# zefanyang/pacingpseudo

Hardware: AMD Instinct MI355X
Metric: training images/sec (256x256, 5-class) (higher is better)
Workload: dtype f32 (matrix products as 3 fp16 MFMA products of split operands with fp32 accumulation, or fp32 MFMA)

## Files before the change

### pacingpseudo_amd/csrc/pp_wino.hip

```cpp
#include "pp_common.h"
#include <stdlib.h>

PP_NS_BEGIN

typedef float f32x16 __attribute__((ext_vector_type(16)));
typedef float f32x4 __attribute__((ext_vector_type(4)));
#define WLD 36
#define WBK 32

struct WinoGeom {
  int N, H, W, dil;
  int Hs, Ws;
  int m;
  int th, tw;
  int T;
  int nb;
};
static inline int wino_tile(int H, int W, int dil) {
  return (H % (4 * dil) == 0 && W % (4 * dil) == 0) ? 4 : 2;
}
static inline WinoGeom wino_geom(int N, int H, int W, int dil) {
  const int m = wino_tile(H, W, dil);
  WinoGeom g{N, H, W, dil, H / dil, W / dil, m, H / dil / m, W / dil / m, 0, (m + 2) * (m + 2)};
  g.T = N * dil * dil * g.th * g.tw;
// ... 707 lines not shown
      U[(r * 4 + 3) * plane + at] = t[r][2];
    }
  }
}

struct GemmArgs {
  const float* A; const float* B; float* C;
  int M, N, K;
  int m_tiles, n_tiles;
  unsigned a_bytes, b_bytes;
  int nb;
};

template <int TM, int TN, int WAVES_M, int WAVES_N>
__global__ __launch_bounds__(WAVES_M* WAVES_N * 64) void wino_gemm_kernel(GemmArgs a) {
  constexpr int NT = WAVES_M * WAVES_N * 64;
  constexpr int BM = 32 * TM * WAVES_M, BN = 32 * TN * WAVES_N;
  constexpr int RPP = NT / 8;
  constexpr int A_PASSES = BM / RPP, B_PASSES = BN / RPP;
  extern __shared__ __attribute__((aligned(16))) float smem[];
  float* As = smem;
  float* Bs = smem + 2 * BM * WLD;
  const int tid = threadIdx.x, lane = tid & 63, wv = tid >> 6;
  const int wm = wv / WAVES_N, wn = wv % WAVES_N;
  const int lr = lane & 31, lh = lane >> 5;
  const int q = tid & 7, r0 = tid >> 3;
  const int per_batch = a.m_tiles * a.n_tiles;
  int b = blockIdx.x;
  const int total = per_batch * a.nb;
  if ((total & 7) == 0) b = (b & 7) * (total >> 3) + (b >> 3);
  const int batch = b / per_batch;
  const int rem = b - batch * per_batch;
  const int mt = rem / a.n_tiles, nt = rem % a.n_tiles;
  const int m0 = mt * BM, n0 = nt * BN;
  const float* Ab = a.A + (size_t)batch * a.M * a.K;
  const float* Bb = a.B + (size_t)batch * a.N * a.K;
  const __amdgpu_buffer_rsrc_t rs_a = __builtin_amdgcn_make_buffer_rsrc((void*)Ab, 0, a.a_bytes, 0x00020000);
  const __amdgpu_buffer_rsrc_t rs_b = __builtin_amdgcn_make_buffer_rsrc((void*)Bb, 0, a.b_bytes, 0x00020000);
  f32x4 ra[A_PASSES], rb[B_PASSES];
  const int n_it = (a.K + WBK - 1) / WBK;
  auto load_tile = [&](int it) {
    const int c = it * WBK + q * 4;
    const int cok = (int)(c < a.K);
#pragma unroll
    for (int i = 0; i < A_PASSES; ++i) {
      const int m = m0 + r0 + i * RPP;
      const unsigned off = (cok & (int)(m < a.M)) ? (unsigned)(m * a.K + c) * 4u : 0xffffffffu;
      ra[i] = __builtin_bit_cast(f32x4, __builtin_amdgcn_raw_buffer_load_b128(rs_a, off, 0, 0));
    }
#pragma unroll
    for (int i = 0; i < B_PASSES; ++i) {
      const int n = n0 + r0 + i * RPP;
      const unsigned off = (cok & (int)(n < a.N)) ? (unsigned)(n * a.K + c) * 4u : 0xffffffffu;
      rb[i] = __builtin_bit_cast(f32x4, __builtin_amdgcn_raw_buffer_load_b128(rs_b, off, 0, 0));
    }
  };
  auto store_tile = [&](int buf) {
#pragma unroll
    for (int i = 0; i < A_PASSES; ++i)
      *reinterpret_cast<f32x4*>(As + buf * BM * WLD + (r0 + i * RPP) * WLD + q * 4) = ra[i];
#pragma unroll
    for (int i = 0; i < B_PASSES; ++i)
      *reinterpret_cast<f32x4*>(Bs + buf * BN * WLD + (r0 + i * RPP) * WLD + q * 4) = rb[i];
  };
  f32x16 acc[TM][TN];
#pragma unroll
  for (int i = 0; i < TM; ++i)
#pragma unroll
    for (int j = 0; j < TN; ++j)
#pragma unroll
      for (int r = 0; r < 16; ++r) acc[i][j][r] = 0.f;
  load_tile(0);
  store_tile(0);
  __syncthreads();
  for (int it = 0; it < n_it; ++it) {
    const int buf = it & 1;
    const bool more = it + 1 < n_it;
    const float* Ap = As + buf * BM * WLD + (wm * TM * 32 + lr) * WLD + lh * 4;
    const float* Bp = Bs + buf * BN * WLD + (wn * TN * 32 + lr) * WLD + lh * 4;
    float4 af[2][TM], bf[2][TN];
    auto read_frags = [&](int kk, int slot) {
#pragma unroll
      for (int i = 0; i < TM; ++i) af[slot][i] = *reinterpret_cast<const float4*>(Ap + i * 32 * WLD + kk * 8);
#pragma unroll
      for (int j = 0; j < TN; ++j) bf[slot][j] = *reinterpret_cast<const float4*>(Bp + j * 32 * WLD + kk * 8);
    };
    auto mfma_block = [&](int slot) {
#pragma unroll
      for (int i = 0; i < TM; ++i)
#pragma unroll
        for (int j = 0; j < TN; ++j) {
          acc[i][j] = __builtin_amdgcn_mfma_f32_32x32x2f32(af[slot][i].x, bf[slot][j].x, acc[i][j], 0, 0, 0);
          acc[i][j] = __builtin_amdgcn_mfma_f32_32x32x2f32(af[slot][i].y, bf[slot][j].y, acc[i][j], 0, 0, 0);
          acc[i][j] = __builtin_amdgcn_mfma_f32_32x32x2f32(af[slot][i].z, bf[slot][j].z, acc[i][j], 0, 0, 0);
          acc[i][j] = __builtin_amdgcn_mfma_f32_32x32x2f32(af[slot][i].w, bf[slot][j].w, acc[i][j], 0, 0, 0);
        }
    };
    read_frags(0, 0);
    read_frags(1, 1);
    __builtin_amdgcn_sched_barrier(0);
    mfma_block(0);
    __builtin_amdgcn_sched_barrier(0);
    if (more) load_tile(it + 1);
    read_frags(2, 0);
    __builtin_amdgcn_sched_barrier(0);
    mfma_block(1);
    __builtin_amdgcn_sched_barrier(0);
    read_frags(3, 1);
    __builtin_amdgcn_sched_barrier(0);
    mfma_block(0);
    __builtin_amdgcn_sched_barrier(0);
    if (more) store_tile(buf ^ 1);
    __builtin_amdgcn_sched_barrier(0);
    mfma_block(1);
    __syncthreads();
  }
  float* Cb = a.C + (size_t)batch * a.M * a.N;
#pragma unroll
  for (int j = 0; j < TN; ++j) {
    const int n = n0 + (wn * TN + j) * 32 + lr;
    if (n >= a.N) continue;
#pragma unroll
    for (int i = 0; i < TM; ++i)
#pragma unroll
      for (int r = 0; r < 16; ++r) {
        const int m = m0 + (wm * TM + i) * 32 + (r & 3) + 8 * (r >> 2) + 4 * lh;
        if (m < a.M) Cb[(size_t)m * a.N + n] = acc[i][j][r];
      }
  }
}

template <int TM, int TN, int WAVES_M, int WAVES_N>
static int launch_gemm(GemmArgs a, hipStream_t s) {
  constexpr int BM = 32 * TM * WAVES_M, BN = 32 * TN * WAVES_N;
  a.m_tiles = pp_cdiv(a.M, BM);
  a.n_tiles = pp_cdiv(a.N, BN);
  const size_t lds = (size_t)2 * (BM + BN) * WLD * sizeof(float);
  auto kern = wino_gemm_kernel<TM, TN, WAVES_M, WAVES_N>;
  {
    pp_max_lds(reinterpret_cast<const void*>(kern), (int)lds);
  }
  hipLaunchKernelGGL(kern, dim3(a.nb * a.m_tiles * a.n_tiles), dim3(WAVES_M * WAVES_N * 64), lds, s, a);
  return pp_launch_status("wino_gemm");
}

struct GemmPsArgs {
  const char* A; const char* B; float* C;
  int M, N, K;
  int m_tiles, n_tiles, nb;
  unsigned a_bytes, b_bytes;
  const float* a_amax; float a_bound;
};

__device__ __forceinline__ f32x16 ps_mfma(f16x8 a, f16x8 b, f32x16 c, int) { return __builtin_amdgcn_mfma_f32_32x32x16_f16(a, b, c, 0, 0, 0); }

template <int TM, int TN, int WAVES_M, int WAVES_N, bool X1>
__global__ __launch_bounds__(WAVES_M* WAVES_N * 64) __attribute__((amdgpu_waves_per_eu(WAVES_M* WAVES_N / 4)))
void wino_gemm_ps_kernel(GemmPsArgs a) {
  constexpr int NW = WAVES_M * WAVES_N;
  constexpr int BM = 32 * TM * WAVES_M, BN = 32 * TN * WAVES_N;
  constexpr int STAGE = (BM + BN) * 128;
  constexpr int FA = BM / 8 / NW, FB = BN / 8 / NW;
  static_assert((BM / 8) % NW == 0 && (BN / 8) % NW == 0, "tile rows must split evenly over the waves");
  extern __shared__ __attribute__((aligned(1024))) char smem_ps[];
  typedef __attribute__((address_space(3))) void* lds_ptr;
  const int tid = threadIdx.x, lane = tid & 63;
  const int wv = __builtin_amdgcn_readfirstlane(tid >> 6);
  const int wm = wv / WAVES_N, wn = wv % WAVES_N;
  const int lr = lane & 31, lh = lane >> 5;
  const int per_batch = a.m_tiles * a.n_tiles;
  int b = blockIdx.x;
  const int total = per_batch * a.nb;
  if ((total & 7) == 0) b = (b & 7) * (total >> 3) + (b >> 3);
  const int batch = b / per_batch;
  const int rem = b - batch * per_batch;
  const int mt = rem / a.n_tiles, nt = rem % a.n_tiles;
  const int m0 = mt * BM, n0 = nt * BN;
  float s_in, s_out;
  ps_scales(a.a_amax, a.a_bound, s_in, s_out);
  const __amdgpu_buffer_rsrc_t rs_a = __builtin_amdgcn_make_buffer_rsrc((void*)(a.A + (size_t)batch * a.a_bytes), 0, a.a_bytes, 0x00020000);
  const __amdgpu_buffer_rsrc_t rs_b = __builtin_amdgcn_make_buffer_rsrc((void*)(a.B + (size_t)batch * a.b_bytes), 0, a.b_bytes, 0x00020000);
  const int fr = lane >> 3, fq = lane & 7;
  const unsigned kbytes = (unsigned)a.K * 4u;
  unsigned offA[FA], offB[FB], pcA[FA], pcB[FB];
#pragma unroll
  for (int f = 0; f < FA; ++f) {
    const int row = (f * NW + wv) * 8 + fr;
    pcA[f] = (unsigned)((fq ^ ((row >> 1) & 7)) * 16);
    offA[f] = (m0 + row < a.M) ? (unsigned)(m0 + row) * kbytes + pcA[f] : 0xffffffffu;
  }
#pragma unroll
  for (int f = 0; f < FB; ++f) {
    const int row = (f * NW + wv) * 8 + fr;
    pcB[f] = (unsigned)((fq ^ ((row >> 1) & 7)) * 16);
    offB[f] = (n0 + row < a.N) ? (unsigned)(n0 + row) * kbytes + pcB[f] : 0xffffffffu;
  }
  auto fill_one = [&](int f, int it, int stage) {
    char* base = smem_ps + stage * STAGE + wv * 1024;
    const unsigned koff = (unsigned)it * 128u;
    if (f < FA) {
      const unsigned o = (offA[f < FA ? f : 0] != 0xffffffffu && koff + pcA[f < FA ? f : 0] < kbytes) ? offA[f < FA ? f : 0] + koff : 0xffffffffu;
      __builtin_amdgcn_raw_ptr_buffer_load_lds(rs_a, (lds_ptr)(base + f * NW * 1024), 16, o, 0, 0, 0);
    } else {
      const int g = f - FA < FB ? f - FA : 0;
      const unsigned o = (offB[g] != 0xffffffffu && koff + pcB[g] < kbytes) ? offB[g] + koff : 0xffffffffu;
      __builtin_amdgcn_raw_ptr_buffer_load_lds(rs_b, (lds_ptr)(base + BM * 128 + g * NW * 1024), 16, o, 0, 0, 0);
    }
  };
  auto fill = [&](int it, int stage) {
#pragma unroll
    for (int f = 0; f < FA + FB; ++f) fill_one(f, it, stage);
  };
  f32x16 accm[TM][TN], accc[TM][TN];
#pragma unroll
  for (int i = 0; i < TM; ++i)
#pragma unroll
    for (int j = 0; j < TN; ++j)
#pragma unroll
      for (int r = 0; r < 16; ++r) { accm[i][j][r] = 0.f; accc[i][j][r] = 0.f; }
  const int sw = (lr >> 1) & 7;
  int qo[2][2];
#pragma unroll
  for (int kb = 0; kb < 2; ++kb)
#pragma unroll
    for (int part = 0; part < 2; ++part) qo[kb][part] = ((4 * kb + 2 * lh + part) ^ sw) * 16;
  const int a_row = (wm * TM * 32 + lr) * 128, b_row = BM * 128 + (wn * TN * 32 + lr) * 128;
  const int n_it = (a.K + 31) / 32;
  f16x8 ah[2][TM], al[2][TM], bh[2][TN], bl[2][TN];
  auto read_half = [&](int kb, int stage) {
    const char* Ap = smem_ps + stage * STAGE + a_row;
    const char* Bp = smem_ps + stage * STAGE + b_row;
#pragma unroll
    for (int i = 0; i < TM; ++i) {
      ah[kb][i] = *reinterpret_cast<const f16x8*>(Ap + i * 32 * 128 + qo[kb][0]);
      if (!X1) al[kb][i] = *reinterpret_cast<const f16x8*>(Ap + i * 32 * 128 + qo[kb][1]);
    }
#pragma unroll
    for (int j = 0; j < TN; ++j) {
      bh[kb][j] = *reinterpret_cast<const f16x8*>(Bp + j * 32 * 128 + qo[kb][0]);
      if (!X1) bl[kb][j] = *reinterpret_cast<const f16x8*>(Bp + j * 32 * 128 + qo[kb][1]);
    }
  };
  auto wait_landed = [&]() {
    asm volatile("s_waitcnt vmcnt(%0) lgkmcnt(0)" ::"n"(FA + FB) : "memory");
    __builtin_amdgcn_s_barrier();
    asm volatile("" ::: "memory");
  };
  static_assert(FA + FB <= 16, "the counted wait assumes a handful of DMAs per wave and stage");
  fill(0, 0);
  fill(1, 1);
  asm volatile("s_waitcnt vmcnt(%0)" ::"n"(FA + FB) : "memory");
  __builtin_amdgcn_s_barrier();
  asm volatile("" ::: "memory");
  fill(2, 2);
  read_half(0, 0);
  read_half(1, 0);
  int st_next = 1, st_free = 0;
  for (int it = 0; it < n_it; ++it) {
    __builtin_amdgcn_sched_barrier(0);
#pragma unroll
    for (int i = 0; i < TM; ++i)
#pragma unroll
      for (int j = 0; j < TN; ++j) {
        accm[i][j] = ps_mfma(ah[0][i], bh[0][j], accm[i][j], 0);
        if (!X1) {
          accc[i][j] = ps_mfma(ah[0][i], bl[0][j], accc[i][j], 0);
          accc[i][j] = ps_mfma(al[0][i], bh[0][j], accc[i][j], 0);
        }
      }
    __builtin_amdgcn_sched_barrier(0);
    wait_landed();
    read_half(0, st_next);
    __builtin_amdgcn_sched_barrier(0);
#pragma unroll
    for (int i = 0; i < TM; ++i)
#pragma unroll
      for (int j = 0; j < TN; ++j) {
        accm[i][j] = ps_mfma(ah[1][i], bh[1][j], accm[i][j], 1);
        if (!X1) {
          accc[i][j] = ps_mfma(ah[1][i], bl[1][j], accc[i][j], 1);
          accc[i][j] = ps_mfma(al[1][i], bh[1][j], accc[i][j], 1);
        }
        constexpr int GROUPS = TM * TN;
        const int gidx = i * TN + j;
#pragma unroll
        for (int f = 0; f < FA + FB; ++f)
          if (f * GROUPS / (FA + FB) == gidx) fill_one(f, it + 3, st_free);
        __builtin_amdgcn_sched_barrier(0);
      }
    read_half(1, st_next);
    st_free = st_next;
    st_next = st_next == 2 ? 0 : st_next + 1;
  }
  asm volatile("s_waitcnt vmcnt(0) lgkmcnt(0)" ::: "memory");
  float* Cb = a.C + (size_t)batch * a.M * a.N;
#pragma unroll
  for (int j = 0; j < TN; ++j) {
    const int n = n0 + (wn * TN + j) * 32 + lr;
    if (n >= a.N) continue;
#pragma unroll
    for (int i = 0; i < TM; ++i)
#pragma unroll
      for (int r = 0; r < 16; ++r) {
        const int m = m0 + (wm * TM + i) * 32 + (r & 3) + 8 * (r >> 2) + 4 * lh;
        if (m < a.M) Cb[(size_t)m * a.N + n] = (X1 ? accm[i][j][r] : accm[i][j][r] + accc[i][j][r] * (1.f / F16_LO_SCALE)) * s_out;
      }
  }
}

template <int TM, int TN, int WAVES_M, int WAVES_N, bool X1>
__global__ __launch_bounds__(WAVES_M* WAVES_N * 64) __attribute__((amdgpu_waves_per_eu(WAVES_M* WAVES_N / 4)))
void wino_gemm_psp_kernel(GemmPsArgs a) {
  constexpr int NW = WAVES_M * WAVES_N;
  constexpr int BM = 32 * TM * WAVES_M, BN = 32 * TN * WAVES_N;
  constexpr int STAGE = (BM + BN) * 128;
  constexpr int FA = BM / 8 / NW, FB = BN / 8 / NW;
  static_assert((BM / 8) % NW == 0 && (BN / 8) % NW == 0, "tile rows must split evenly over the waves");
  static_assert(FA + FB <= 16, "the counted wait below assumes a handful of DMAs per wave and stage");
  constexpr int NST = TM * TN * 16;
  constexpr int WIN = NST + FA + FB < 63 ? NST + FA + FB : 63;
  extern __shared__ __attribute__((aligned(1024))) char smem_ps[];
  typedef __attribute__((address_space(3))) void* lds_ptr;
  const int tid = threadIdx.x, lane = tid & 63;
  const int wv = __builtin_amdgcn_readfirstlane(tid >> 6);
  const int wm = wv / WAVES_N, wn = wv % WAVES_N;
  const int lr = lane & 31, lh = lane >> 5;
  const int per_batch = a.m_tiles * a.n_tiles;
  const int total = per_batch * a.nb;
  const int G = (int)gridDim.x;
  const int n_my = ((int)blockIdx.x < total) ? (total - (int)blockIdx.x + G - 1) / G : 0;
  if (n_my == 0) return;
  const bool xcd = (total & 7) == 0 && (G & 7) == 0;
  auto tile_of = [&](int seq, int& batch, int& m0, int& n0) {
    const int it = (int)blockIdx.x + seq * G;
    const int b = xcd ? (it & 7) * (total >> 3) + (it >> 3) : it;
    batch = b / per_batch;
    const int rem = b - batch * per_batch;
    m0 = (rem / a.n_tiles) * BM;
    n0 = (rem % a.n_tiles) * BN;
  };
  float s_in, s_out;
  ps_scales(a.a_amax, a.a_bound, s_in, s_out);
  const int fr = lane >> 3, fq = lane & 7;
  const unsigned kbytes = (unsigned)a.K * 4u;
  const int n_it = (a.K + 31) / 32;
  unsigned pcA[FA], pcB[FB], offA[FA], offB[FB];
#pragma unroll
  for (int f = 0; f < FA; ++f) pcA[f] = (unsigned)((fq ^ ((((f * NW + wv) * 8 + fr) >> 1) & 7)) * 16);
#pragma unroll
  for (int f = 0; f < FB; ++f) pcB[f] = (unsigned)((fq ^ ((((f * NW + wv) * 8 + fr) >> 1) & 7)) * 16);
  int f_seq = 0, f_it = 0, f_batch = 0;
  auto fill_tile = [&](int seq) {
    int m0 = 0, n0 = 0;
    const bool live = seq < n_my;
    if (live) tile_of(seq, f_batch, m0, n0);
#pragma unroll
    for (int f = 0; f < FA; ++f) {
      const int row = (f * NW + wv) * 8 + fr;
      offA[f] = (live && m0 + row < a.M) ? (unsigned)(m0 + row) * kbytes + pcA[f] : 0xffffffffu;
    }
#pragma unroll
    for (int f = 0; f < FB; ++f) {
      const int row = (f * NW + wv) * 8 + fr;
      offB[f] = (live && n0 + row < a.N) ? (unsigned)(n0 + row) * kbytes + pcB[f] : 0xffffffffu;
    }
  };
  fill_tile(0);
  auto fill_one = [&](int f, int stage) {
    const __amdgpu_buffer_rsrc_t rs_a = __builtin_amdgcn_make_buffer_rsrc((void*)(a.A + (size_t)f_batch * a.a_bytes), 0, a.a_bytes, 0x00020000);
    const __amdgpu_buffer_rsrc_t rs_b = __builtin_amdgcn_make_buffer_rsrc((void*)(a.B + (size_t)f_batch * a.b_bytes), 0, a.b_bytes, 0x00020000);
    char* base = smem_ps + stage * STAGE + wv * 1024;
    const unsigned koff = (unsigned)f_it * 128u;
    if (f < FA) {
      const int g = f < FA ? f : 0;
      const unsigned o = (offA[g] != 0xffffffffu && koff + pcA[g] < kbytes) ? offA[g] + koff : 0xffffffffu;
      __builtin_amdgcn_raw_ptr_buffer_load_lds(rs_a, (lds_ptr)(base + g * NW * 1024), 16, o, 0, 0, 0);
    } else {
      const int g = f - FA < FB ? f - FA : 0;
      const unsigned o = (offB[g] != 0xffffffffu && koff + pcB[g] < kbytes) ? offB[g] + koff : 0xffffffffu;
      __builtin_amdgcn_raw_ptr_buffer_load_lds(rs_b, (lds_ptr)(base + BM * 128 + g * NW * 1024), 16, o, 0, 0, 0);
    }
  };
  auto fill_advance = [&]() {
    if (++f_it == n_it) { f_it = 0; ++f_seq; fill_tile(f_seq); }
  };
  auto fill = [&](int stage) {
#pragma unroll
    for (int f = 0; f < FA + FB; ++f) fill_one(f, stage);
    fill_advance();
  };
  f32x16 accm[TM][TN], accc[TM][TN];
#pragma unroll
  for (int i = 0; i < TM; ++i)
#pragma unroll
    for (int j = 0; j < TN; ++j)
#pragma unroll
      for (int r = 0; r < 16; ++r) { accm[i][j][r] = 0.f; accc[i][j][r] = 0.f; }
  const int sw = (lr >> 1) & 7;
  int qo[2][2];
#pragma unroll
  for (int kb = 0; kb < 2; ++kb)
#pragma unroll
    for (int part = 0; part < 2; ++part) qo[kb][part] = ((4 * kb + 2 * lh + part) ^ sw) * 16;
  const int a_row = (wm * TM * 32 + lr) * 128, b_row = BM * 128 + (wn * TN * 32 + lr) * 128;
  f16x8 ah[2][TM], al[2][TM], bh[2][TN], bl[2][TN];
  auto read_half = [&](int kb, int stage) {
    const char* Ap = smem_ps + stage * STAGE + a_row;
    const char* Bp = smem_ps + stage * STAGE + b_row;
#pragma unroll
    for (int i = 0; i < TM; ++i) {
      ah[kb][i] = *reinterpret_cast<const f16x8*>(Ap + i * 32 * 128 + qo[kb][0]);
      if (!X1) al[kb][i] = *reinterpret_cast<const f16x8*>(Ap + i * 32 * 128 + qo[kb][1]);
    }
#pragma unroll
    for (int j = 0; j < TN; ++j) {
      bh[kb][j] = *reinterpret_cast<const f16x8*>(Bp + j * 32 * 128 + qo[kb][0]);
      if (!X1) bl[kb][j] = *reinterpret_cast<const f16x8*>(Bp + j * 32 * 128 + qo[kb][1]);
    }
  };
  int since_store = 2;
  auto wait_landed = [&]() {
    if (since_store < 2) {
      asm volatile("s_waitcnt vmcnt(%0) lgkmcnt(0)" ::"n"(WIN) : "memory");
    } else {
      asm volatile("s_waitcnt vmcnt(%0) lgkmcnt(0)" ::"n"(FA + FB) : "memory");
    }
    __builtin_amdgcn_s_barrier();
    asm volatile("" ::: "memory");
  };
  fill(0);
  fill(1);
  asm volatile("s_waitcnt vmcnt(%0)" ::"n"(FA + FB) : "memory");
  __builtin_amdgcn_s_barrier();
  asm volatile("" ::: "memory");
  fill(2);
  read_half(0, 0);
  read_half(1, 0);
  int st_next = 1, st_free = 0;
  int c_seq = 0, c_it = 0;
  const int total_it = n_my * n_it;
  for (int g = 0; g < total_it; ++g) {
    __builtin_amdgcn_sched_barrier(0);
#pragma unroll
    for (int i = 0; i < TM; ++i)
#pragma unroll
      for (int j = 0; j < TN; ++j) {
        accm[i][j] = ps_mfma(ah[0][i], bh[0][j], accm[i][j], 0);
        if (!X1) {
          accc[i][j] = ps_mfma(ah[0][i], bl[0][j], accc[i][j], 0);
          accc[i][j] = ps_mfma(al[0][i], bh[0][j], accc[i][j], 0);
        }
      }
    __builtin_amdgcn_sched_barrier(0);
    wait_landed();
    ++since_store;
    read_half(0, st_next);
    __builtin_amdgcn_sched_barrier(0);
#pragma unroll
    for (int i = 0; i < TM; ++i)
#pragma unroll
      for (int j = 0; j < TN; ++j) {
        accm[i][j] = ps_mfma(ah[1][i], bh[1][j], accm[i][j], 1);
        if (!X1) {
          accc[i][j] = ps_mfma(ah[1][i], bl[1][j], accc[i][j], 1);
          accc[i][j] = ps_mfma(al[1][i], bh[1][j], accc[i][j], 1);
        }
        constexpr int GROUPS = TM * TN;
        const int gidx = i * TN + j;
#pragma unroll
        for (int f = 0; f < FA + FB; ++f)
          if (f * GROUPS / (FA + FB) == gidx) fill_one(f, st_free);
        __builtin_amdgcn_sched_barrier(0);
      }
    fill_advance();
    read_half(1, st_next);
    st_free = st_next;
    st_next = st_next == 2 ? 0 : st_next + 1;
    if (++c_it == n_it) {
      int batch, m0, n0;
      tile_of(c_seq, batch, m0, n0);
      float* Cb = a.C + (size_t)batch * a.M * a.N;
#pragma unroll
      for (int j = 0; j < TN; ++j) {
        const int n = n0 + (wn * TN + j) * 32 + lr;
#pragma unroll
        for (int i = 0; i < TM; ++i)
#pragma unroll
          for (int r = 0; r < 16; ++r) {
            const int m = m0 + (wm * TM + i) * 32 + (r & 3) + 8 * (r >> 2) + 4 * lh;
            const float v = (X1 ? accm[i][j][r] : accm[i][j][r] + accc[i][j][r] * (1.f / F16_LO_SCALE)) * s_out;
            Cb[(size_t)m * a.N + n] = v;
            accm[i][j][r] = 0.f; accc[i][j][r] = 0.f;
          }
      }
      c_it = 0; ++c_seq; since_store = 0;
    }
  }
  asm volatile("s_waitcnt vmcnt(0) lgkmcnt(0)" ::: "memory");
}

template <int TM, int TN, int WAVES_M, int WAVES_N, bool X1>
static int launch_gemm_ps(GemmPsArgs a, hipStream_t s) {
  constexpr int BM = 32 * TM * WAVES_M, BN = 32 * TN * WAVES_N;
  a.m_tiles = pp_cdiv(a.M, BM);
  a.n_tiles = pp_cdiv(a.N, BN);
  const size_t lds = (size_t)3 * (BM + BN) * 128;
  auto kern = wino_gemm_ps_kernel<TM, TN, WAVES_M, WAVES_N, X1>;
  pp_max_lds(reinterpret_cast<const void*>(kern), (int)lds);
  static const int persist = getenv("PP_WINO_GEMM_PERSIST") ? atoi(getenv("PP_WINO_GEMM_PERSIST")) : 1;
  const int total = a.nb * a.m_tiles * a.n_tiles;
  if (persist && a.M % BM == 0 && a.N % BN == 0 && a.K >= 128 && total >= 2 * 256) {
    auto kp = wino_gemm_psp_kernel<TM, TN, WAVES_M, WAVES_N, X1>;
    pp_max_lds(reinterpret_cast<const void*>(kp), (int)lds);
    hipLaunchKernelGGL(kp, dim3(256), dim3(WAVES_M * WAVES_N * 64), lds, s, a);
    return pp_launch_status("wino_gemm_psp");
  }
  hipLaunchKernelGGL(kern, dim3(total), dim3(WAVES_M * WAVES_N * 64), lds, s, a);
  return pp_launch_status("wino_gemm_ps");
}
template <bool X1>
static int launch_gemm_ps_any(const GemmPsArgs& a, hipStream_t s) {
  if (a.N % 256 == 0) return launch_gemm_ps<2, 2, 2, 4, X1>(a, s);
  if (a.N % 128 == 0) return launch_gemm_ps<2, 2, 4, 2, X1>(a, s);
  return launch_gemm_ps<2, 1, 4, 2, X1>(a, s);
}

static inline int wino_blocks(long long total) {
  int b = pp_cdiv(total, 256);
  return b > 16384 ? 16384 : (b < 1 ? 1 : b);
}

static int wino_check(int C, int N, int B, int H, int W, int dil) {
  PP_CHECK_ARG(dil >= 1 && H % (2 * dil) == 0 && W % (2 * dil) == 0, "winograd: H, W must be multiples of 2*dilation");
  PP_CHECK_ARG(C % 4 == 0 && N % 4 == 0 && C > 0 && N > 0 && B > 0, "winograd: channel counts must be multiples of 4");
  const long long T = (long long)B * H * W / 4;
  PP_CHECK_ARG(T * C < 0x3fffffffLL && T * N < 0x3fffffffLL && (long long)N * C < 0x3fffffffLL,
               "winograd: plane exceeds the 4 GiB buffer-descriptor range");
  return 0;
}

#ifndef PP_ACT_16
extern "C" size_t pp_conv3x3_wino_workspace(int Cin, int Cout, int B, int H, int W, int dil) {
  const WinoGeom g = wino_geom(B, H, W, dil);
  return (size_t)g.nb * g.T * ((size_t)Cin + Cout) * sizeof(float) + 256;
}

extern "C" size_t pp_conv3x3_wino_vkeep_elems(int Cin, int B, int H, int W, int dil) {
  const WinoGeom g = wino_geom(B, H, W, dil);
  return (size_t)g.nb * g.T * Cin + 4;
}

extern "C" int pp_conv3x3_wino_tile(int H, int W, int dil) { return wino_tile(H, W, dil); }

extern "C" int pp_wino_pack_weights(const float* w_oihw, int O, int I, int tile, float* Uf, float* Ub, void* stream) {
  PP_CHECK_ARG(w_oihw && (Uf || Ub) && (tile == 2 || tile == 4), "wino_pack_weights: bad arguments");
  if (tile == 2)
    hipLaunchKernelGGL(wino_weight_kernel, dim3(pp_cdiv((long long)O * I, 256)), dim3(256), 0, (hipStream_t)stream,
                       w_oihw, O, I, Uf, Ub);
  else
    hipLaunchKernelGGL(wino4_weight_kernel, dim3(pp_cdiv((long long)O * I, 256)), dim3(256), 0, (hipStream_t)stream,
                       w_oihw, O, I, Uf, Ub);
  return pp_launch_status("wino_pack_weights");
}
#endif

static int wino_own_amax(const act_t* x, int ld, int C, long long P, float* slot, hipStream_t s) {
  if (hipMemsetAsync(slot, 0, sizeof(float), s) != hipSuccess) return pp_launch_status("wino_amax_memset");
  hipLaunchKernelGGL(wino_amax_kernel, dim3(wino_blocks(P * (C / 4))), dim3(256), 0, s, x, ld, C, P, slot);
  return pp_launch_status("wino_amax");
}

static int wino_conv(const act_t* in, int ld_in, int C, const float* U, const float* bias, act_t* out, int ld_out, int N,
                     int B, int H, int W, int dil, int accumulate, float* v_keep, void* ws, size_t ws_bytes,
                     hipStream_t s, bool f16 = false, PpEpi* epi = nullptr, bool* fused = nullptr,
                     const float* in_amax = nullptr, bool own_amax = false) {
  if (fused) *fused = false;
  if (int rc = wino_check(C, N, B, H, W, dil)) return rc;
  PP_CHECK_ARG(in && U && out && ws, "winograd conv: null pointer");
  PP_CHECK_ARG(ld_in % 4 == 0 && ld_out % 4 == 0 && ld_in >= C && ld_out >= N, "winograd conv: bad ld");
  WinoGeom g = wino_geom(B, H, W, dil);
  const size_t need = (size_t)g.nb * g.T * ((v_keep ? 0 : (size_t)C) + N) * sizeof(float) + (f16 ? 16 : 0);
  if (ws_bytes < need) {
    pp_set_error("winograd conv: workspace too small (%zu < %zu)", ws_bytes, need);
    return PP_ERR_WORKSPACE;
  }
  PP_CHECK_ARG(!f16 || (g.m == 4 && C % 8 == 0), "winograd f16x3: only the F(4x4,3x3) geometry (H, W multiples of 4*dilation) with K %% 8 == 0");
  PP_CHECK_ARG(!f16 || ((((uintptr_t)in & PP_ACT_ALIGN) | ((uintptr_t)U & 15)) == 0), "winograd f16x3: in / U must be 16-byte aligned");
#ifdef PP_ACT_16
  if (!f16) { pp_set_error("winograd conv (16-bit storage): only the split-fp16 F(4x4,3x3) path exists"); return PP_ERR_UNSUPPORTED; }
#endif
  if (f16 && own_amax && !in_amax) {
    float* slot = reinterpret_cast<float*>(reinterpret_cast<char*>(ws) + ((need - 16 + 15) & ~(size_t)15));
    if (int rc = wino_own_amax(in, ld_in, C, (long long)B * H * W, slot, s)) return rc;
    in_amax = slot;
  }
  float* V = v_keep ? v_keep : reinterpret_cast<float*>(ws);
  float* M = v_keep ? reinterpret_cast<float*>(ws) : V + (size_t)g.nb * g.T * C;
  const double P = (double)B * H * W;
  const double expand = (double)g.nb / (g.m * g.m);
  pp_prof_begin(PP_K_WINO_XFORM, 0.0, 4.0 * P * C * (1.0 + expand), s);
#ifdef PP_ACT_16
  launch_wino4_input_ps(in, ld_in, C, g, reinterpret_cast<char*>(V), in_amax, s);
#else
  if (g.m == 2)
    hipLaunchKernelGGL(wino_input_kernel, dim3(wino_blocks((long long)g.T * (C / 4))), dim3(256), 0, s, in, ld_in, C, g, V);
  else if (f16)
    launch_wino4_input_ps(in, ld_in, C, g, reinterpret_cast<char*>(V), in_amax, s);
  else
    WINO4_LAUNCH(wino4_input_kernel, wino4_vec(in, ld_in, C), (long long)g.T * C, s, in, ld_in, C, g, V, (float*)nullptr);
#endif
  pp_prof_end(s);
  if (int rc = pp_launch_status("wino_input")) return rc;
  int rc;
  if (f16) {
    pp_prof_begin2(PP_K_WINO_GEMM_F16X3, 6.0 * expand * P * (double)N * C, 18.0 * P * (double)N * C,
                   4.0 * (P * C + P * N + 9.0 * C * N), s);
    GemmPsArgs ga{reinterpret_cast<const char*>(V), reinterpret_cast<const char*>(U), M, g.T, N, C, 0, 0, g.nb,
                  (unsigned)((size_t)g.T * C * 4), (unsigned)((size_t)N * C * 4), in_amax, PS_BOUND_INPUT};
    rc = pp_f16_products() == 1 ? launch_gemm_ps_any<true>(ga, s) : launch_gemm_ps_any<false>(ga, s);
  } else {
    GemmArgs ga{V, U, M, g.T, N, C, 0, 0, (unsigned)((size_t)g.T * C * 4), (unsigned)((size_t)N * C * 4), g.nb};
    pp_prof_begin2(PP_K_WINO_GEMM, 2.0 * expand * P * (double)N * C, 18.0 * P * (double)N * C,
                   4.0 * (P * C + P * N + 9.0 * C * N), s);
    rc = (N % 128 == 0) ? launch_gemm<2, 2, 2, 2>(ga, s) : launch_gemm<2, 1, 2, 2>(ga, s);
  }
  pp_prof_end(s);
  if (rc) return rc;
  pp_prof_begin(PP_K_WINO_XFORM, 0.0, 4.0 * P * N * (1.0 + expand), s);
#ifndef PP_ACT_16
  if (g.m == 2) {
    hipLaunchKernelGGL(wino_output_kernel, dim3(wino_blocks((long long)g.T * (N / 4))), dim3(256), 0, s, M, N, g, bias,
                       out, ld_out, accumulate);
  } else
#endif
  {
    const int vec = (bias && ((uintptr_t)bias & 15)) ? 1 : wino4_vec(out, ld_out, N);
    const int cv = N / vec;
    const bool can_fuse = epi && epi->mode && fused && !accumulate && epi->groups <= PP_EPI_GROUPS &&
                          (256 % cv == 0 || cv % 256 == 0) && epi->px_per_group % (H * W) == 0 &&
                          (epi->mode != 2 || ((((uintptr_t)epi->scale | (uintptr_t)epi->shift) & 15) == 0));
    if (can_fuse) {
      const int unit = cv > 256 ? cv / 256 : 1;
      int blocks = wino_blocks((long long)g.T * cv);
      if (blocks > 512) blocks = 512;
      blocks = (blocks + unit - 1) / unit * unit;
      epi->rows = blocks / unit;
      const int ipg = epi->px_per_group / (H * W);
// ... 634 lines not shown
```

Baseline: 1102.

## Switch Winograd split-fp16 GEMM to 16x16x32 MFMA with interleaved LDS reads

Replaces the 32x32x16 MFMA core of the split-precision Winograd GEMM kernels with 16x16x32 MFMA tiles, held in a shared PsCore helper. The LDS swizzle is changed to suit the new fragment access pattern. The K-step now interleaves next-stage LDS fragment reads and DMA fills between rows of MFMAs, instead of double-buffering half-K fragment sets. The aim is to cut register pressure and hide LDS latency better, at the cost of more, smaller MFMA instructions and a more rigid schedule (static_assert SM==4).

```diff
diff --git a/pacingpseudo_amd/csrc/pp_wino.hip b/pacingpseudo_amd/csrc/pp_wino.hip
--- a/pacingpseudo_amd/csrc/pp_wino.hip
+++ b/pacingpseudo_amd/csrc/pp_wino.hip
@@ -883,7 +883,136 @@
   const float* a_amax; float a_bound;
 };
 
-__device__ __forceinline__ f32x16 ps_mfma(f16x8 a, f16x8 b, f32x16 c, int) { return __builtin_amdgcn_mfma_f32_32x32x16_f16(a, b, c, 0, 0, 0); }
+__device__ __forceinline__ int ps_swz(int row) {
+  const int j = (row >> 1) & 7;
+  return 2 * (j & 3) + (j >> 2);
+}
+__device__ __forceinline__ f32x4 ps_mfma(f16x8 a, f16x8 b, f32x4 c) { return __builtin_amdgcn_mfma_f32_16x16x32_f16(a, b, c, 0, 0, 0); }
+
+template <int TM, int TN, bool X1>
+struct PsCore {
+  static constexpr int SM = 2 * TM, SN = 2 * TN;
+  static constexpr int NPH = X1 ? 1 : 3;
+  static constexpr int NSLOT = (SM - 2) * NPH;
+  static_assert(SM >= 3 && SN % 2 == 0, "the K-step below needs middle rows for the DMAs and column pairs");
+  f32x4 accm[SM][SN], accc[SM][SN];
+  f16x8 fa[SM][2], fb[SN][2];
+  int a_off, b_off, q[2];
+
+  __device__ __forceinline__ void init(int lane, int wm, int wn, int BM) {
+    const int ll = lane & 15, lq = lane >> 4;
+    a_off = (wm * TM * 32 + ll) * 128;
+    b_off = BM * 128 + (wn * TN * 32 + ll) * 128;
+    q[0] = ((2 * lq) ^ ps_swz(ll)) * 16;
+    q[1] = ((2 * lq + 1) ^ ps_swz(ll)) * 16;
+    clear();
+  }
+  __device__ __forceinline__ void clear() {
+#pragma unroll
+    for (int i = 0; i < SM; ++i)
+#pragma unroll
+      for (int j = 0; j < SN; ++j)
+#pragma unroll
+        for (int r = 0; r < 4; ++r) { accm[i][j][r] = 0.f; accc[i][j][r] = 0.f; }
+  }
+  template <int I, int PART>
+  __device__ __forceinline__ void read_a(const char* stage) {
+    fa[I][PART] = *reinterpret_cast<const f16x8*>(stage + a_off + I * 16 * 128 + q[PART]);
+  }
+  template <int J, int PART>
+  __device__ __forceinline__ void read_b(const char* stage) {
+    fb[J][PART] = *reinterpret_cast<const f16x8*>(stage + b_off + J * 16 * 128 + q[PART]);
+  }
+  template <int I>
+  __device__ __forceinline__ void read_a_sub(const char* stage) {
+    read_a<I, 0>(stage);
+    if (!X1) read_a<I, 1>(stage);
+  }
+  __device__ __forceinline__ void read_all(const char* stage) {
+    read_a_sub<0>(stage);
+    read_a_sub<1>(stage);
+    if (SM > 2) { read_a_sub<SM - 2>(stage); read_a_sub<SM - 1>(stage); }
+#pragma unroll
+    for (int j = 0; j < SN; ++j) {
+      fb[j][0] = *reinterpret_cast<const f16x8*>(stage + b_off + j * 16 * 128 + q[0]);
+      if (!X1) fb[j][1] = *reinterpret_cast<const f16x8*>(stage + b_off + j * 16 * 128 + q[1]);
+    }
+  }
+  template <int I, int J, int PH>
+  __device__ __forceinline__ void prod() {
+    if (PH == 0) accm[I][J] = ps_mfma(fa[I][0], fb[J][0], accm[I][J]);
+    if (PH == 1) accc[I][J] = ps_mfma(fa[I][1], fb[J][0], accc[I][J]);
+    if (PH == 2) accc[I][J] = ps_mfma(fa[I][0], fb[J][1], accc[I][J]);
+  }
+  template <int I, int PH>
+  __device__ __forceinline__ void phase() {
+    prod<I, 0, PH>();
+    prod<I, 1, PH>();
+    if (SN > 2) { prod<I, SN - 2, PH>(); prod<I, SN - 1, PH>(); }
+  }
+  template <int I, int SLOT0, int NF, class Fill>
+  __device__ __forceinline__ void row_fill(Fill&& fill_one) {
+    auto fills = [&](int slot) {
+#pragma unroll
+      for (int f = 0; f < NF; ++f)
+        if (f * NSLOT / NF == slot) fill_one(f);
+      __builtin_amdgcn_sched_barrier(0);
+    };
+    phase<I, 0>();
+    fills(SLOT0);
+    if (!X1) {
+      phase<I, 1>();
+      fills(SLOT0 + 1);
+      phase<I, 2>();
+      fills(SLOT0 + 2);
+    }
+  }
+  template <int J>
+  __device__ __forceinline__ void last_pair(const char* nxt) {
+    constexpr int I = SM - 1;
+    prod<I, J, 0>();
+    prod<I, J + 1, 0>();
+    if (!X1) {
+      prod<I, J, 1>();
+      prod<I, J + 1, 1>();
+    }
+    __builtin_amdgcn_sched_barrier(0);
+    read_b<J, 0>(nxt);
+    read_b<J + 1, 0>(nxt);
+    __builtin_amdgcn_sched_barrier(0);
+    if (!X1) {
+      prod<I, J, 2>();
+      prod<I, J + 1, 2>();
+      __builtin_amdgcn_sched_barrier(0);
+      read_b<J, 1>(nxt);
+      read_b<J + 1, 1>(nxt);
+      __builtin_amdgcn_sched_barrier(0);
+    }
+  }
+  template <int NF, class Wait, class Fill>
+  __device__ __forceinline__ void kstep(const char* nxt, Wait&& wait_landed, Fill&& fill_one) {
+    static_assert(SM == 4, "rows 1 and 2 carry the DMAs");
+    __builtin_amdgcn_sched_barrier(0);
+    phase<0, 0>();
+    if (!X1) { phase<0, 1>(); phase<0, 2>(); }
+    __builtin_amdgcn_sched_barrier(0);
+    wait_landed();
+    read_a_sub<0>(nxt);
+    __builtin_amdgcn_sched_barrier(0);
+    row_fill<1, 0, NF>(fill_one);
+    read_a_sub<1>(nxt);
+    __builtin_amdgcn_sched_barrier(0);
+    row_fill<2, NPH, NF>(fill_one);
+    read_a_sub<2>(nxt);
+    __builtin_amdgcn_sched_barrier(0);
+    last_pair<0>(nxt);
+    if (SN > 2) last_pair<SN - 2>(nxt);
+    read_a_sub<3>(nxt);
+  }
+  __device__ __forceinline__ float value(int i, int j, int r, float s_out) const {
+    return (X1 ? accm[i][j][r] : accm[i][j][r] + accc[i][j][r] * (1.f / F16_LO_SCALE)) * s_out;
+  }
+};
 
 template <int TM, int TN, int WAVES_M, int WAVES_N, bool X1>
 __global__ __launch_bounds__(WAVES_M* WAVES_N * 64) __attribute__((amdgpu_waves_per_eu(WAVES_M* WAVES_N / 4)))
@@ -898,7 +1027,7 @@
   const int tid = threadIdx.x, lane = tid & 63;
   const int wv = __builtin_amdgcn_readfirstlane(tid >> 6);
   const int wm = wv / WAVES_N, wn = wv % WAVES_N;
-  const int lr = lane & 31, lh = lane >> 5;
+  const int ll = lane & 15, lq = lane >> 4;
   const int per_batch = a.m_tiles * a.n_tiles;
   int b = blockIdx.x;
   const int total = per_batch * a.nb;
@@ -917,13 +1046,13 @@
 #pragma unroll
   for (int f = 0; f < FA; ++f) {
     const int row = (f * NW + wv) * 8 + fr;
-    pcA[f] = (unsigned)((fq ^ ((row >> 1) & 7)) * 16);
+    pcA[f] = (unsigned)((fq ^ ps_swz(row)) * 16);
     offA[f] = (m0 + row < a.M) ? (unsigned)(m0 + row) * kbytes + pcA[f] : 0xffffffffu;
   }
 #pragma unroll
   for (int f = 0; f < FB; ++f) {
     const int row = (f * NW + wv) * 8 + fr;
-    pcB[f] = (unsigned)((fq ^ ((row >> 1) & 7)) * 16);
+    pcB[f] = (unsigned)((fq ^ ps_swz(row)) * 16);
     offB[f] = (n0 + row < a.N) ? (unsigned)(n0 + row) * kbytes + pcB[f] : 0xffffffffu;
   }
   auto fill_one = [&](int f, int it, int stage) {
@@ -942,36 +1071,9 @@
 #pragma unroll
     for (int f = 0; f < FA + FB; ++f) fill_one(f, it, stage);
   };
-  f32x16 accm[TM][TN], accc[TM][TN];
-#pragma unroll
-  for (int i = 0; i < TM; ++i)
-#pragma unroll
-    for (int j = 0; j < TN; ++j)
-#pragma unroll
-      for (int r = 0; r < 16; ++r) { accm[i][j][r] = 0.f; accc[i][j][r] = 0.f; }
-  const int sw = (lr >> 1) & 7;
-  int qo[2][2];
-#pragma unroll
-  for (int kb = 0; kb < 2; ++kb)
-#pragma unroll
-    for (int part = 0; part < 2; ++part) qo[kb][part] = ((4 * kb + 2 * lh + part) ^ sw) * 16;
-  const int a_row = (wm * TM * 32 + lr) * 128, b_row = BM * 128 + (wn * TN * 32 + lr) * 128;
+  PsCore<TM, TN, X1> core;
+  core.init(lane, wm, wn, BM);
   const int n_it = (a.K + 31) / 32;
-  f16x8 ah[2][TM], al[2][TM], bh[2][TN], bl[2][TN];
-  auto read_half = [&](int kb, int stage) {
-    const char* Ap = smem_ps + stage * STAGE + a_row;
-    const char* Bp = smem_ps + stage * STAGE + b_row;
-#pragma unroll
-    for (int i = 0; i < TM; ++i) {
-      ah[kb][i] = *reinterpret_cast<const f16x8*>(Ap + i * 32 * 128 + qo[kb][0]);
-      if (!X1) al[kb][i] = *reinterpret_cast<const f16x8*>(Ap + i * 32 * 128 + qo[kb][1]);
-    }
-#pragma unroll
-    for (int j = 0; j < TN; ++j) {
-      bh[kb][j] = *reinterpret_cast<const f16x8*>(Bp + j * 32 * 128 + qo[kb][0]);
-      if (!X1) bl[kb][j] = *reinterpret_cast<const f16x8*>(Bp + j * 32 * 128 + qo[kb][1]);
-    }
-  };
   auto wait_landed = [&]() {
     asm volatile("s_waitcnt vmcnt(%0) lgkmcnt(0)" ::"n"(FA + FB) : "memory");
     __builtin_amdgcn_s_barrier();
@@ -984,57 +1086,25 @@
   __builtin_amdgcn_s_barrier();
   asm volatile("" ::: "memory");
   fill(2, 2);
-  read_half(0, 0);
-  read_half(1, 0);
-  int st_next = 1, st_free = 0;
+  core.read_all(smem_ps);
+  int st_cur = 0, st_next = 1;
   for (int it = 0; it < n_it; ++it) {
-    __builtin_amdgcn_sched_barrier(0);
-#pragma unroll
-    for (int i = 0; i < TM; ++i)
-#pragma unroll
-      for (int j = 0; j < TN; ++j) {
-        accm[i][j] = ps_mfma(ah[0][i], bh[0][j], accm[i][j], 0);
-        if (!X1) {
-          accc[i][j] = ps_mfma(ah[0][i], bl[0][j], accc[i][j], 0);
-          accc[i][j] = ps_mfma(al[0][i], bh[0][j], accc[i][j], 0);
-        }
-      }
-    __builtin_amdgcn_sched_barrier(0);
-    wait_landed();
-    read_half(0, st_next);
-    __builtin_amdgcn_sched_barrier(0);
-#pragma unroll
-    for (int i = 0; i < TM; ++i)
-#pragma unroll
-      for (int j = 0; j < TN; ++j) {
-        accm[i][j] = ps_mfma(ah[1][i], bh[1][j], accm[i][j], 1);
-        if (!X1) {
-          accc[i][j] = ps_mfma(ah[1][i], bl[1][j], accc[i][j], 1);
-          accc[i][j] = ps_mfma(al[1][i], bh[1][j], accc[i][j], 1);
-        }
-        constexpr int GROUPS = TM * TN;
-        const int gidx = i * TN + j;
-#pragma unroll
-        for (int f = 0; f < FA + FB; ++f)
-          if (f * GROUPS / (FA + FB) == gidx) fill_one(f, it + 3, st_free);
-        __builtin_amdgcn_sched_barrier(0);
-      }
-    read_half(1, st_next);
-    st_free = st_next;
+    core.template kstep<FA + FB>(smem_ps + st_next * STAGE, wait_landed, [&](int f) { fill_one(f, it + 3, st_cur); });
+    st_cur = st_next;
     st_next = st_next == 2 ? 0 : st_next + 1;
   }
   asm volatile("s_waitcnt vmcnt(0) lgkmcnt(0)" ::: "memory");
   float* Cb = a.C + (size_t)batch * a.M * a.N;
 #pragma unroll
-  for (int j = 0; j < TN; ++j) {
-    const int n = n0 + (wn * TN + j) * 32 + lr;
+  for (int j = 0; j < 2 * TN; ++j) {
+    const int n = n0 + wn * TN * 32 + j * 16 + ll;
     if (n >= a.N) continue;
 #pragma unroll
-    for (int i = 0; i < TM; ++i)
-#pragma unroll
-      for (int r = 0; r < 16; ++r) {
-        const int m = m0 + (wm * TM + i) * 32 + (r & 3) + 8 * (r >> 2) + 4 * lh;
-        if (m < a.M) Cb[(size_t)m * a.N + n] = (X1 ? accm[i][j][r] : accm[i][j][r] + accc[i][j][r] * (1.f / F16_LO_SCALE)) * s_out;
+    for (int i = 0; i < 2 * TM; ++i)
+#pragma unroll
+      for (int r = 0; r < 4; ++r) {
+        const int m = m0 + wm * TM * 32 + i * 16 + 4 * lq + r;
+        if (m < a.M) Cb[(size_t)m * a.N + n] = core.value(i, j, r, s_out);
       }
   }
 }
@@ -1055,7 +1125,7 @@
   const int tid = threadIdx.x, lane = tid & 63;
   const int wv = __builtin_amdgcn_readfirstlane(tid >> 6);
   const int wm = wv / WAVES_N, wn = wv % WAVES_N;
-  const int lr = lane & 31, lh = lane >> 5;
+  const int ll = lane & 15, lq = lane >> 4;
   const int per_batch = a.m_tiles * a.n_tiles;
   const int total = per_batch * a.nb;
   const int G = (int)gridDim.x;
@@ -1077,9 +1147,9 @@
   const int n_it = (a.K + 31) / 32;
   unsigned pcA[FA], pcB[FB], offA[FA], offB[FB];
 #pragma unroll
-  for (int f = 0; f < FA; ++f) pcA[f] = (unsigned)((fq ^ ((((f * NW + wv) * 8 + fr) >> 1) & 7)) * 16);
-#pragma unroll
-  for (int f = 0; f < FB; ++f) pcB[f] = (unsigned)((fq ^ ((((f * NW + wv) * 8 + fr) >> 1) & 7)) * 16);
+  for (int f = 0; f < FA; ++f) pcA[f] = (unsigned)((fq ^ ps_swz((f * NW + wv) * 8 + fr)) * 16);
+#pragma unroll
+  for (int f = 0; f < FB; ++f) pcB[f] = (unsigned)((fq ^ ps_swz((f * NW + wv) * 8 + fr)) * 16);
   int f_seq = 0, f_it = 0, f_batch = 0;
   auto fill_tile = [&](int seq) {
     int m0 = 0, n0 = 0;
@@ -1120,35 +1190,8 @@
     for (int f = 0; f < FA + FB; ++f) fill_one(f, stage);
     fill_advance();
   };
-  f32x16 accm[TM][TN], accc[TM][TN];
-#pragma unroll
-  for (int i = 0; i < TM; ++i)
-#pragma unroll
-    for (int j = 0; j < TN; ++j)
-#pragma unroll
-      for (int r = 0; r < 16; ++r) { accm[i][j][r] = 0.f; accc[i][j][r] = 0.f; }
-  const int sw = (lr >> 1) & 7;
-  int qo[2][2];
-#pragma unroll
-  for (int kb = 0; kb < 2; ++kb)
-#pragma unroll
-    for (int part = 0; part < 2; ++part) qo[kb][part] = ((4 * kb + 2 * lh + part) ^ sw) * 16;
-  const int a_row = (wm * TM * 32 + lr) * 128, b_row = BM * 128 + (wn * TN * 32 + lr) * 128;
-  f16x8 ah[2][TM], al[2][TM], bh[2][TN], bl[2][TN];
-  auto read_half = [&](int kb, int stage) {
-    const char* Ap = smem_ps + stage * STAGE + a_row;
-    const char* Bp = smem_ps + stage * STAGE + b_row;
-#pragma unroll
-    for (int i = 0; i < TM; ++i) {
-      ah[kb][i] = *reinterpret_cast<const f16x8*>(Ap + i * 32 * 128 + qo[kb][0]);
-      if (!X1) al[kb][i] = *reinterpret_cast<const f16x8*>(Ap + i * 32 * 128 + qo[kb][1]);
-    }
-#pragma unroll
-    for (int j = 0; j < TN; ++j) {
-      bh[kb][j] = *reinterpret_cast<const f16x8*>(Bp + j * 32 * 128 + qo[kb][0]);
-      if (!X1) bl[kb][j] = *reinterpret_cast<const f16x8*>(Bp + j * 32 * 128 + qo[kb][1]);
-    }
-  };
+  PsCore<TM, TN, X1> core;
+  core.init(lane, wm, wn, BM);
   int since_store = 2;
   auto wait_landed = [&]() {
     if (since_store < 2) {
@@ -1158,6 +1201,7 @@
     }
     __builtin_amdgcn_s_barrier();
     asm volatile("" ::: "memory");
+    ++since_store;
   };
   fill(0);
   fill(1);
@@ -1165,65 +1209,31 @@
   __builtin_amdgcn_s_barrier();
   asm volatile("" ::: "memory");
   fill(2);
-  read_half(0, 0);
-  read_half(1, 0);
-  int st_next = 1, st_free = 0;
+  core.read_all(smem_ps);
+  int st_cur = 0, st_next = 1;
   int c_seq = 0, c_it = 0;
   const int total_it = n_my * n_it;
   for (int g = 0; g < total_it; ++g) {
-    __builtin_amdgcn_sched_barrier(0);
-#pragma unroll
-    for (int i = 0; i < TM; ++i)
-#pragma unroll
-      for (int j = 0; j < TN; ++j) {
-        accm[i][j] = ps_mfma(ah[0][i], bh[0][j], accm[i][j], 0);
-        if (!X1) {
-          accc[i][j] = ps_mfma(ah[0][i], bl[0][j], accc[i][j], 0);
-          accc[i][j] = ps_mfma(al[0][i], bh[0][j], accc[i][j], 0);
-        }
-      }
-    __builtin_amdgcn_sched_barrier(0);
-    wait_landed();
-    ++since_store;
-    read_half(0, st_next);
-    __builtin_amdgcn_sched_barrier(0);
-#pragma unroll
-    for (int i = 0; i < TM; ++i)
-#pragma unroll
-      for (int j = 0; j < TN; ++j) {
-        accm[i][j] = ps_mfma(ah[1][i], bh[1][j], accm[i][j], 1);
-        if (!X1) {
-          accc[i][j] = ps_mfma(ah[1][i], bl[1][j], accc[i][j], 1);
-          accc[i][j] = ps_mfma(al[1][i], bh[1][j], accc[i][j], 1);
-        }
-        constexpr int GROUPS = TM * TN;
-        const int gidx = i * TN + j;
-#pragma unroll
-        for (int f = 0; f < FA + FB; ++f)
-          if (f * GROUPS / (FA + FB) == gidx) fill_one(f, st_free);
-        __builtin_amdgcn_sched_barrier(0);
-      }
+    core.template kstep<FA + FB>(smem_ps + st_next * STAGE, wait_landed, [&](int f) { fill_one(f, st_cur); });
     fill_advance();
-    read_half(1, st_next);
-    st_free = st_next;
+    st_cur = st_next;
     st_next = st_next == 2 ? 0 : st_next + 1;
     if (++c_it == n_it) {
       int batch, m0, n0;
       tile_of(c_seq, batch, m0, n0);
       float* Cb = a.C + (size_t)batch * a.M * a.N;
 #pragma unroll
-      for (int j = 0; j < TN; ++j) {
-        const int n = n0 + (wn * TN + j) * 32 + lr;
-#pragma unroll
-        for (int i = 0; i < TM; ++i)
-#pragma unroll
-          for (int r = 0; r < 16; ++r) {
-            const int m = m0 + (wm * TM + i) * 32 + (r & 3) + 8 * (r >> 2) + 4 * lh;
-            const float v = (X1 ? accm[i][j][r] : accm[i][j][r] + accc[i][j][r] * (1.f / F16_LO_SCALE)) * s_out;
-            Cb[(size_t)m * a.N + n] = v;
-            accm[i][j][r] = 0.f; accc[i][j][r] = 0.f;
+      for (int j = 0; j < 2 * TN; ++j) {
+        const int n = n0 + wn * TN * 32 + j * 16 + ll;
+#pragma unroll
+        for (int i = 0; i < 2 * TM; ++i)
+#pragma unroll
+          for (int r = 0; r < 4; ++r) {
+            const int m = m0 + wm * TM * 32 + i * 16 + 4 * lq + r;
+            Cb[(size_t)m * a.N + n] = core.value(i, j, r, s_out);
           }
       }
+      core.clear();
       c_it = 0; ++c_seq; since_store = 0;
     }
   }
```

Result: slower. 1088 (-1.2%).
